# KohakuBlueleaf/UwUDiff

Measured on AMD Instinct MI355X. Metric: train images/sec (whole node), DiT-S/2 256^2 latent, higher is better.
Workload: dtype bf16; 1 GPU; DiT-S/2 (L12 D384 h6), 4x32x32 synthetic latents + pooled-text cond 1280, eps-MSE, AdamW lr1e-6 wd0.01 cosine; random-init weights; per_gpu_batch=768, global_batch=768, parallelism=dp1

## Files before the change

uwudiff_amd/csrc/attention_p256.hip:

```cpp
#include "common.h"

namespace {

constexpr int P_RING = 3;
template <int DH>
struct PGeom {
  static constexpr bool TAIL = DH > 64;
  static constexpr int SLOT = 16384 + (TAIL ? 2048 + 256 : 0);
  static constexpr int OFF_TT = 16384, OFF_TL = 16384 + 2048;
  static constexpr int OFF_DS = P_RING * SLOT;
  static constexpr int KIMG = 32768 + (TAIL ? 4096 : 0);
  static constexpr int OFF_K = OFF_DS + 32768;
  static constexpr int OFF_LSE = OFF_K + 2 * KIMG;
  static constexpr int OFF_DELTA = OFF_LSE + (TAIL ? 0 : 2 * 1024);
  static constexpr int OFF_ZERO = OFF_DELTA + 2 * 256;
  static constexpr int LDS = OFF_ZERO + (TAIL ? 16 : 0);
};
static_assert(PGeom<64>::LDS == 150016 && PGeom<72>::LDS <= 163840, "LDS budget");
constexpr int P_LDS = PGeom<64>::LDS;

struct PArgs {
  const bf16_t *q, *k, *v, *o, *dO;
  bf16_t *dq, *dk, *dv;
  const float* lse;
  int B, H, ldq, ldk, ldv, ldo, nheads;
  float scale;
};

__device__ __forceinline__ int fsw(int row) {
  return (((row >> 2) ^ (row >> 4)) & 1) | ((((row >> 3) ^ (row >> 4)) & 1) << 1) | (((row >> 1) & 1) << 2);
}
__device__ __forceinline__ int Fsw(int row) {
  return (row & 1) | (((row >> 2) & 1) << 1) | (((row >> 3) & 1) << 2) | (((row >> 1) & 1) << 3);
}

typedef short s16x4 __attribute__((ext_vector_type(4)));
typedef unsigned su32x2 __attribute__((ext_vector_type(2)));

__device__ __forceinline__ void glds16(const void* gsrc, unsigned lds_dst ) {
  unsigned keep;
  asm volatile("s_mov_b32 %0, m0\n\ts_mov_b32 m0, %2\n\ts_nop 0\n\tglobal_load_lds_dwordx4 %1, off\n\ts_mov_b32 m0, %0"
               : "=&s"(keep)
               : "v"(gsrc), "s"(lds_dst)
               : "memory");
}
__device__ __forceinline__ void glds4(const void* gsrc, unsigned lds_dst ) {
  unsigned keep;
  asm volatile("s_mov_b32 %0, m0\n\ts_mov_b32 m0, %2\n\ts_nop 0\n\tglobal_load_lds_dword %1, off\n\ts_mov_b32 m0, %0"
               : "=&s"(keep)
               : "v"(gsrc), "s"(lds_dst)
               : "memory");
}
__device__ __forceinline__ void glds16_s(const void* sbase , unsigned voff, unsigned lds_dst ) {
  unsigned keep;
  asm volatile("s_mov_b32 %0, m0\n\ts_mov_b32 m0, %3\n\ts_nop 0\n\tglobal_load_lds_dwordx4 %1, %2\n\ts_mov_b32 m0, %0"
               : "=&s"(keep)
               : "v"(voff), "s"(sbase), "s"(lds_dst)
               : "memory");
}
__device__ __forceinline__ f32x16 mfma32(const uint4& a, const uint4& b, f32x16 c) {
  return __builtin_amdgcn_mfma_f32_32x32x16_bf16(*reinterpret_cast<const bf16x8*>(&a), *reinterpret_cast<const bf16x8*>(&b), c, 0,
                                                 0, 0);
}
__device__ __forceinline__ f32x4 mfma16(const uint4& a, const uint4& b, f32x4 c) {
  return __builtin_amdgcn_mfma_f32_16x16x32_bf16(*reinterpret_cast<const bf16x8*>(&a), *reinterpret_cast<const bf16x8*>(&b), c, 0,
                                                 0, 0);
}
__device__ __forceinline__ uint4 pack8(const f32x16& x, int s) {
  bf16x8 f;
#pragma unroll
  for (int j = 0; j < 8; ++j) f[j] = (bf16_t)x[8 * s + j];
  return *reinterpret_cast<uint4*>(&f);
}

extern __shared__ __attribute__((aligned(16))) char p_smem[];

__device__ __forceinline__ void lane_halves(float x, float& lo, float& hi) {
  float a = x, b = x;
  asm volatile("v_nop\n\tv_nop\n\tv_permlane32_swap_b32 %0, %1" : "+v"(a), "+v"(b));
  lo = a;
  hi = b;
}

__device__ __forceinline__ uint4 tr_pair(unsigned a0, unsigned a1) {
  const s16x4 lo = __builtin_amdgcn_ds_read_tr16_b64_v4i16(
      (__attribute__((address_space(3))) s16x4*)((__attribute__((address_space(3))) char*)p_smem + a0));
  const s16x4 hi = __builtin_amdgcn_ds_read_tr16_b64_v4i16(
      (__attribute__((address_space(3))) s16x4*)((__attribute__((address_space(3))) char*)p_smem + a1));
  uint4 r;
  r.x = ((unsigned)(unsigned short)lo[0]) | ((unsigned)(unsigned short)lo[1] << 16);
  r.y = ((unsigned)(unsigned short)lo[2]) | ((unsigned)(unsigned short)lo[3] << 16);
  r.z = ((unsigned)(unsigned short)hi[0]) | ((unsigned)(unsigned short)hi[1] << 16);
  r.w = ((unsigned)(unsigned short)hi[2]) | ((unsigned)(unsigned short)hi[3] << 16);
  return r;
}

template <int DH>
__global__ void __launch_bounds__(512, 2) attn_bwd_p256(const PArgs a) {
  using G = PGeom<DH>;
  constexpr bool TAIL = G::TAIL;
  constexpr int T = 256, NKS = TAIL ? 5 : 4, NDT = TAIL ? 3 : 2;
  constexpr int P_SLOT = G::SLOT, P_OFF_DS = G::OFF_DS, P_OFF_K = G::OFF_K, P_OFF_LSE = G::OFF_LSE, P_OFF_DELTA = G::OFF_DELTA;
  constexpr int KIMG = G::KIMG;
  char* const smem = p_smem;
  const int tid = threadIdx.x, lane = tid & 63;
  const int wave = __builtin_amdgcn_readfirstlane(tid >> 6);
  const int r = lane & 31, h = lane >> 5;
  const int fr = lane & 15, fq = lane >> 4;
  const unsigned smem_base = (unsigned)(size_t)((const __attribute__((address_space(3))) char*)p_smem);
  const float c = a.scale * 1.4426950408889634f;
  const float ninv_scale = -1.f / a.scale;
  const int nmy = (a.nheads - (int)blockIdx.x + (int)gridDim.x - 1) / (int)gridDim.x;
  const int total = 4 * nmy;
  const int k0 = wave * 32;

  const int drow = tid >> 3;
  const int dchunk = (tid & 7) ^ fsw(drow);
  unsigned B0, A0, K0, D0, TQ0, TA0, KT0;
  auto phase1_consts = [&](int ln) {
    const int r_ = ln & 31, h_ = ln >> 5;
    B0 = (unsigned)(r_ * 128 + ((h_ ^ fsw(r_)) << 4));
    const int rowL = 4 * h_ + ((ln & 15) >> 2), chunkL = 2 * ((ln >> 4) & 1) + ((ln & 3) >> 1);
    A0 = (unsigned)(rowL * 128 + ((chunkL ^ fsw(rowL)) << 4) + 8 * (ln & 1));
    TQ0 = (unsigned)((r_ >> 3) * 256 + (r_ & 7) * 16);
    TA0 = (unsigned)(rowL * 16 + 8 * (ln & 1));
  };
  auto phase2_consts = [&](int ln) {
    const int fr_ = ln & 15, fq_ = ln >> 4;
    const int rowK = 8 * fq_ + (fr_ >> 2);
    K0 = (unsigned)(rowK * 128 + ((((fr_ & 3) >> 1) ^ fsw(rowK)) << 4) + 8 * (fr_ & 1));
    D0 = (unsigned)(rowK * 128 + (((fr_ & 3) ^ Fsw(rowK)) << 3));
    KT0 = (unsigned)(rowK * 16 + 8 * (fr_ & 1));
  };
  auto opaque_lane = [&]() {
    int ln = lane;
    asm volatile("" : "+v"(ln));
    return ln;
  };
  auto my_tid = [&]() {
    int x = tid;
    if constexpr (TAIL) asm volatile("" : "+v"(x));
    return x;
  };
  if constexpr (!TAIL) {
    phase1_consts(lane);
    phase2_consts(lane);
  }

  auto head_ptrs = [&](int j, int& b, int& hd) {
    const int bh = (int)blockIdx.x + j * (int)gridDim.x;
    b = bh / a.H;
    hd = bh - b * a.H;
  };
  uint4 oreg;
  unsigned otail = 0;
  auto issue_tile = [&](int g) {
    int b, hd;
    head_ptrs(g >> 2, b, hd);
    const int tid = my_tid(), lane = tid & 63, drow = tid >> 3, dchunk = (tid & 7) ^ fsw(drow);
    const int row = 64 * (g & 3) + drow;
    const bf16_t* qs = a.q + ((int64_t)b * T + row) * a.ldq + hd * DH + 8 * dchunk;
    const bf16_t* gs = a.dO + ((int64_t)b * T + row) * a.ldo + hd * DH + 8 * dchunk;
    const unsigned dst = smem_base + (unsigned)((g % P_RING) * P_SLOT + wave * 1024);
    glds16(qs, dst);
    glds16(gs, dst + 8192);
    oreg = *reinterpret_cast<const uint4*>(a.o + ((int64_t)b * T + row) * a.ldo + hd * DH + 8 * dchunk);
    if constexpr (TAIL) {
      const unsigned slot = smem_base + (unsigned)((g % P_RING) * P_SLOT);
      if (lane < 16) {
        const int64_t trow = (int64_t)b * T + 64 * (g & 3) + 8 * wave + (lane & 7);
        const bf16_t* src = lane < 8 ? a.q + trow * a.ldq + hd * DH + 64 : a.dO + trow * a.ldo + hd * DH + 64;
        glds16(src, slot + (unsigned)(G::OFF_TT + wave * 256));
      }
      glds4(a.lse + ((int64_t)b * a.H + hd) * T + 64 * (g & 3) + lane, slot + (unsigned)G::OFF_TL);
      otail = *reinterpret_cast<const unsigned*>(a.o + ((int64_t)b * T + row) * a.ldo + hd * DH + 64 + 2 * (tid & 3));
    }
  };
  auto issue_head = [&](int j) {
    int b, hd;
    head_ptrs(j, b, hd);
    const int tid = my_tid(), lane = tid & 63, drow = tid >> 3, dchunk = (tid & 7) ^ fsw(drow);
    const unsigned dst = smem_base + (unsigned)(P_OFF_K + (j & 1) * KIMG + wave * 1024);
#pragma unroll
    for (int p = 0; p < 4; ++p)
      glds16(a.k + ((int64_t)b * T + 64 * p + drow) * a.ldk + hd * DH + 8 * dchunk, dst + p * 8192);
    if constexpr (TAIL) {
      if (lane < 32)
        glds16(a.k + ((int64_t)b * T + 32 * wave + lane) * a.ldk + hd * DH + 64,
               smem_base + (unsigned)(P_OFF_K + (j & 1) * KIMG + 32768 + wave * 512));
    } else {
      glds4(a.lse + ((int64_t)b * a.H + hd) * T + 64 * (wave & 3) + lane,
            smem_base + (unsigned)(P_OFF_LSE + (j & 1) * 1024 + (wave & 3) * 256));
    }
  };
  uint4 kf[NKS], vf[NKS];
  auto load_kv = [&](int j) {
    int b, hd;
    head_ptrs(j, b, hd);
    const int tid = my_tid(), r = tid & 31, h = (tid >> 5) & 1;
#pragma unroll
    for (int s = 0; s < 4; ++s) {
      kf[s] = *reinterpret_cast<const uint4*>(a.k + ((int64_t)b * T + k0 + r) * a.ldk + hd * DH + 16 * s + 8 * h);
      vf[s] = *reinterpret_cast<const uint4*>(a.v + ((int64_t)b * T + k0 + r) * a.ldv + hd * DH + 16 * s + 8 * h);
    }
    if constexpr (TAIL) {
      kf[4] = *reinterpret_cast<const uint4*>(a.k + ((int64_t)b * T + k0 + r) * a.ldk + hd * DH + 64);
      vf[4] = *reinterpret_cast<const uint4*>(a.v + ((int64_t)b * T + k0 + r) * a.ldv + hd * DH + 64);
    }
  };
  auto delta_of = [&](int g) {
    const uint4 gch = *reinterpret_cast<const uint4*>(smem + (g % P_RING) * P_SLOT + 8192 + 16 * tid);
    const bf16x8 gv = *reinterpret_cast<const bf16x8*>(&gch), ov = *reinterpret_cast<const bf16x8*>(&oreg);
    float ds = 0.f;
#pragma unroll
    for (int e = 0; e < 8; ++e) ds += (float)gv[e] * (float)ov[e];
    if constexpr (TAIL) {
      const unsigned gtc = *reinterpret_cast<const unsigned*>(smem + (g % P_RING) * P_SLOT + G::OFF_TT + (drow >> 3) * 256 + 128 +
                                                              (drow & 7) * 16 + 4 * (tid & 3));
      const bf16x2 gt2 = *reinterpret_cast<const bf16x2*>(&gtc), ot2 = *reinterpret_cast<const bf16x2*>(&otail);
      const float dt2 = (float)gt2[0] * (float)ot2[0] + (float)gt2[1] * (float)ot2[1];
      ds += (tid & 4) ? 0.f : dt2;
    }
    ds += __builtin_bit_cast(float, __builtin_amdgcn_update_dpp(0, __builtin_bit_cast(int, ds), 0xB1, 0xF, 0xF, true));
    ds += __builtin_bit_cast(float, __builtin_amdgcn_update_dpp(0, __builtin_bit_cast(int, ds), 0x4E, 0xF, 0xF, true));
    ds += __builtin_bit_cast(float, __builtin_amdgcn_update_dpp(0, __builtin_bit_cast(int, ds), 0x141, 0xF, 0xF, true));
    if ((tid & 7) == 0) reinterpret_cast<float*>(smem + P_OFF_DELTA + (g & 1) * 256)[drow] = -ds;
  };

  f32x16 dkT[2], dvT[2];
  f32x4 dkt = {0.f, 0.f, 0.f, 0.f}, dvt = {0.f, 0.f, 0.f, 0.f};
#pragma unroll
  for (int dt = 0; dt < 2; ++dt) dkT[dt] = dvT[dt] = f32x16{};

  auto store_dkdv = [&](int j) {
    int b, hd;
    head_ptrs(j, b, hd);
    const int tid = my_tid(), lane = tid & 63, r = tid & 31, h = (tid >> 5) & 1;
    char* mine = smem + P_OFF_K + (j & 1) * KIMG + wave * 4096;
    char* mine_t = smem + P_OFF_K + (j & 1) * KIMG + 32768 + wave * 512;
#pragma unroll
    for (int which = 0; which < 2; ++which) {
#pragma unroll
      for (int dt = 0; dt < 2; ++dt)
#pragma unroll
        for (int g4 = 0; g4 < 4; ++g4) {
          const int d0 = 32 * dt + 8 * g4 + 4 * h;
          const f32x16& x = which ? dvT[dt] : dkT[dt];
          const float sc = which ? 1.f : a.scale;
          store4(reinterpret_cast<bf16_t*>(mine + r * 128 + (((d0 >> 3) ^ (r & 7)) << 4) + 2 * (d0 & 7)),
                 f32x4{x[4 * g4] * sc, x[4 * g4 + 1] * sc, x[4 * g4 + 2] * sc, x[4 * g4 + 3] * sc});
        }
      bf16_t* dst = (which ? a.dv : a.dk) + (int64_t)b * T * (which ? a.ldv : a.ldk) + hd * DH;
      const int ld = which ? a.ldv : a.ldk;
#pragma unroll
      for (int p = 0; p < 4; ++p) {
        const int key = 8 * p + (lane >> 3), ch = lane & 7;
        const uint4 x = *reinterpret_cast<const uint4*>(mine + key * 128 + ((ch ^ (key & 7)) << 4));
        *reinterpret_cast<uint4*>(dst + (int64_t)(k0 + key) * ld + 8 * ch) = x;
      }
      if constexpr (TAIL) {
        const f32x4 x = which ? dvt : dkt;
        const float sc = which ? 1.f : a.scale;
        store4(reinterpret_cast<bf16_t*>(mine_t + r * 16 + 8 * h), f32x4{x[0] * sc, x[1] * sc, x[2] * sc, x[3] * sc});
        const uint4 xt = *reinterpret_cast<const uint4*>(mine_t + r * 16);
        *reinterpret_cast<uint4*>(dst + (int64_t)(k0 + r) * ld + 64) = xt;
      }
    }
#pragma unroll
    for (int dt = 0; dt < 2; ++dt) dkT[dt] = dvT[dt] = f32x16{};
    dkt = dvt = f32x4{0.f, 0.f, 0.f, 0.f};
  };

  if (total == 0) return;
  if constexpr (TAIL)
    if (tid < 4) reinterpret_cast<unsigned*>(smem + G::OFF_ZERO)[tid] = 0u;
  issue_head(0);
  issue_tile(0);
  load_kv(0);
  __builtin_amdgcn_s_waitcnt(0x0070);
  asm volatile("" ::: "memory");
  __builtin_amdgcn_s_barrier();
  delta_of(0);
  if (1 < total) issue_tile(1);
  __builtin_amdgcn_s_waitcnt(0x0070);
  for (int g = 0; g < total; ++g) {
    const int j = g >> 2, t = g & 3;
    __builtin_amdgcn_s_waitcnt(TAIL ? 0x0072 : 0x0071);
    asm volatile("" ::: "memory");
    __builtin_amdgcn_s_barrier();
    if (t == 0 && j > 0) store_dkdv(j - 1);
    if (g + 1 < total) delta_of(g + 1);
    if (g + 2 < total) {
      issue_tile(g + 2);
      if (((g + 2) & 3) == 0) issue_head((g + 2) >> 2);
    }
    if constexpr (TAIL) phase1_consts(opaque_lane());
    const unsigned Qs = (unsigned)((g % P_RING) * P_SLOT), Gs = Qs + 8192;
    const float* ls = TAIL ? reinterpret_cast<const float*>(smem + (g % P_RING) * P_SLOT + G::OFF_TL)
                           : reinterpret_cast<const float*>(smem + P_OFF_LSE + (j & 1) * 1024) + 64 * t;
    const float* dl = reinterpret_cast<const float*>(smem + P_OFF_DELTA + (g & 1) * 256);
    char* const dsimg = smem + P_OFF_DS;
#pragma unroll
    for (int sub = 0; sub < 2; ++sub) {
      f32x16 S, dP;
#pragma unroll
      for (int g4 = 0; g4 < 4; ++g4) {
        const f32x4 l4 = load4(ls + 32 * sub + 8 * g4 + 4 * h);
        const f32x4 d4 = load4(dl + 32 * sub + 8 * g4 + 4 * h);
#pragma unroll
        for (int e = 0; e < 4; ++e) {
          S[4 * g4 + e] = l4[e] * ninv_scale;
          dP[4 * g4 + e] = d4[e];
        }
      }
#pragma unroll
      for (int s = 0; s < 4; ++s) {
        const unsigned off = (B0 ^ (unsigned)(s << 5)) + 4096u * sub;
        const uint4 qa = *reinterpret_cast<const uint4*>(smem + Qs + off);
        const uint4 ga = *reinterpret_cast<const uint4*>(smem + Gs + off);
        S = mfma32(qa, kf[s], S);
        dP = mfma32(ga, vf[s], dP);
      }
      if constexpr (TAIL) {
        const unsigned off = Qs + (unsigned)G::OFF_TT + TQ0 + 1024u * sub;
        const uint4 qa = *reinterpret_cast<const uint4*>(smem + (h ? (unsigned)G::OFF_ZERO : off));
        const uint4 ga = *reinterpret_cast<const uint4*>(smem + (h ? (unsigned)G::OFF_ZERO : off + 128));
        S = mfma32(qa, kf[4], S);
        dP = mfma32(ga, vf[4], dP);
      }
#pragma unroll
      for (int i = 0; i < 16; ++i) {
        const float p = __builtin_amdgcn_exp2f(S[i] * c);
        S[i] = p;
        dP[i] *= p;
      }
      bf16x2 dsp[8];
#pragma unroll
      for (int jj = 0; jj < 8; ++jj) dsp[jj] = bf16x2{(bf16_t)dP[2 * jj], (bf16_t)dP[2 * jj + 1]};
#pragma unroll
      for (int g4 = 0; g4 < 4; ++g4) {
        uint2 w;
        w.x = *reinterpret_cast<const unsigned*>(&dsp[2 * g4]);
        w.y = *reinterpret_cast<const unsigned*>(&dsp[2 * g4 + 1]);
        const int key = k0 + r;
        *reinterpret_cast<uint2*>(dsimg + key * 128 + (((8 * sub + 2 * g4 + h) ^ Fsw(key)) << 3)) = w;
      }
      f32x16 tv = {}, tk = {};
#pragma unroll
      for (int s2 = 0; s2 < 2; ++s2) {
        const uint4 pf = pack8(S, s2);
        uint4 dsf;
        dsf.x = *reinterpret_cast<const unsigned*>(&dsp[4 * s2]);
        dsf.y = *reinterpret_cast<const unsigned*>(&dsp[4 * s2 + 1]);
        dsf.z = *reinterpret_cast<const unsigned*>(&dsp[4 * s2 + 2]);
        dsf.w = *reinterpret_cast<const unsigned*>(&dsp[4 * s2 + 3]);
#pragma unroll
        for (int dt = 0; dt < 2; ++dt) {
          const unsigned x0 = (A0 ^ (unsigned)(0x30 * s2) ^ (unsigned)(0x40 * dt)) + 2048u * s2 + 4096u * sub;
          const unsigned x1 = (x0 ^ 0x20u) + 1024u;
          const uint4 gt = tr_pair(Gs + x0, Gs + x1);
          const uint4 qt = tr_pair(Qs + x0, Qs + x1);
          dvT[dt] = mfma32(gt, pf, dvT[dt]);
          dkT[dt] = mfma32(qt, dsf, dkT[dt]);
        }
        if constexpr (TAIL) {
          const unsigned x0 = Qs + (unsigned)G::OFF_TT + TA0 + 512u * s2 + 1024u * sub;
          const uint4 gt = tr_pair(x0 + 128u, x0 + 128u + 256u);
          const uint4 qt = tr_pair(x0, x0 + 256u);
          tv = mfma32(gt, pf, tv);
          tk = mfma32(qt, dsf, tk);
        }
      }
      if constexpr (TAIL) {
#pragma unroll
        for (int e = 0; e < 4; ++e) {
          dvt[e] += tv[e];
          dkt[e] += tk[e];
        }
      }
    }
    if (t == 3 && j + 1 < nmy) load_kv(j + 1);
    asm volatile("s_waitcnt lgkmcnt(0)" ::: "memory");
    __builtin_amdgcn_s_barrier();
    if constexpr (TAIL) phase2_consts(opaque_lane());
    const int qblk = wave & 3, db0 = 2 * (wave >> 2);
    const unsigned Ki = (unsigned)(P_OFF_K + (j & 1) * KIMG), Di = (unsigned)P_OFF_DS;
    const unsigned ka = K0 ^ (unsigned)(db0 << 5), kb = K0 ^ (unsigned)((db0 + 1) << 5), da = D0 ^ (unsigned)(qblk << 5);
    f32x4 acc0 = {0.f, 0.f, 0.f, 0.f}, acc1 = {0.f, 0.f, 0.f, 0.f}, acc2 = {0.f, 0.f, 0.f, 0.f};
#pragma unroll
    for (int kk = 0; kk < 8; ++kk) {
      const unsigned ko = 4096u * kk;
      const uint4 fa = tr_pair(Ki + ka + ko, Ki + (ka ^ 0x10u) + 512u + ko);
      const uint4 fb = tr_pair(Ki + kb + ko, Ki + (kb ^ 0x10u) + 512u + ko);
      const uint4 fd = tr_pair(Di + da + ko, Di + (da ^ 0x10u) + 512u + ko);
      acc0 = mfma16(fa, fd, acc0);
      acc1 = mfma16(fb, fd, acc1);
      if constexpr (TAIL) {
        const unsigned kt = Ki + 32768u + KT0 + 512u * kk;
        acc2 = mfma16(tr_pair(kt, kt + 64u), fd, acc2);
      }
    }
    int b, hd;
    head_ptrs(j, b, hd);
    const f32x4 v0 = acc0 * a.scale, v1 = acc1 * a.scale;
    const bf16x4 p0b = {(bf16_t)v0[0], (bf16_t)v0[1], (bf16_t)v0[2], (bf16_t)v0[3]};
    const bf16x4 p1b = {(bf16_t)v1[0], (bf16_t)v1[1], (bf16_t)v1[2], (bf16_t)v1[3]};
    const uint2 p0 = *reinterpret_cast<const uint2*>(&p0b), p1 = *reinterpret_cast<const uint2*>(&p1b);
    const su32x2 sx = __builtin_amdgcn_permlane16_swap(p0.x, p1.x, false, false);
    const su32x2 sy = __builtin_amdgcn_permlane16_swap(p0.y, p1.y, false, false);
    const bool odd = fq & 1;
    const int d = odd ? 16 * (db0 + 1) + 4 * (fq - 1) : 16 * db0 + 4 * fq;
    bf16_t* dst = a.dq + ((int64_t)b * T + 64 * t + 16 * qblk + fr) * a.ldq + hd * DH + d;
    *reinterpret_cast<uint4*>(dst) = uint4{sx[0], sy[0], sx[1], sy[1]};
    if constexpr (TAIL) {
      const f32x4 v2 = acc2 * a.scale;
      store4(a.dq + ((int64_t)b * T + 64 * t + 16 * qblk + fr) * a.ldq + hd * DH + 64 + 4 * (fq & 1), v2);
    }
  }
  asm volatile("s_waitcnt lgkmcnt(0)" ::: "memory");
  __builtin_amdgcn_s_barrier();
  store_dkdv(nmy - 1);
}

template <int DH>
struct FGeom {
  static constexpr bool TAIL = DH > 64;
  static constexpr int RING = TAIL ? 4 : 5;
  static constexpr int SLOT = 16384 + (TAIL ? 2048 : 0);
  static constexpr int OFF_TT = 16384;
  static constexpr int OST = 4096 + (TAIL ? 512 : 0);
  static constexpr int OFF_O = RING * SLOT;
  static constexpr int OFF_Q = OFF_O + 8 * OST;
  static constexpr int OFF_ZERO = OFF_Q + 32768 + (TAIL ? 4096 : 0);
  static constexpr int LDS = OFF_ZERO + (TAIL ? 16 : 0);
};
static_assert(FGeom<64>::LDS == 147456 && FGeom<72>::LDS <= 163840, "LDS budget");
constexpr int F_LDS = FGeom<64>::LDS;

struct FArgs {
  const bf16_t *q, *k, *v;
  bf16_t* out;
  float* lse;
  int B, H, ldq, ldk, ldv, ldo, nheads;
  float scale;
};

template <int N>
__device__ __forceinline__ void wait_vm_n() {
  asm volatile("s_waitcnt vmcnt(%0)" ::"n"(N) : "memory");
}
__device__ __forceinline__ void wait_vm(int n) {
  switch (n < 20 ? n : 20) {
    case 20: wait_vm_n<20>(); break;
    case 19: wait_vm_n<19>(); break;
    case 18: wait_vm_n<18>(); break;
    case 17: wait_vm_n<17>(); break;
    case 16: wait_vm_n<16>(); break;
    case 15: wait_vm_n<15>(); break;
    case 14: wait_vm_n<14>(); break;
    case 13: wait_vm_n<13>(); break;
    case 12: wait_vm_n<12>(); break;
    case 11: wait_vm_n<11>(); break;
    case 10: wait_vm_n<10>(); break;
    case 9: wait_vm_n<9>(); break;
    case 8: wait_vm_n<8>(); break;
    case 7: wait_vm_n<7>(); break;
    case 6: wait_vm_n<6>(); break;
    case 5: wait_vm_n<5>(); break;
    case 4: wait_vm_n<4>(); break;
    case 3: wait_vm_n<3>(); break;
    case 2: wait_vm_n<2>(); break;
    case 1: wait_vm_n<1>(); break;
    default: wait_vm_n<0>();
  }
}

template <int DH>
__global__ void __launch_bounds__(512, 2) attn_fwd_p256(const FArgs a) {
  using G = FGeom<DH>;
  constexpr bool TAIL = G::TAIL;
  constexpr int T = 256, NKS = TAIL ? 5 : 4, NDT = TAIL ? 3 : 2;
  constexpr int F_RING = G::RING, AHEAD = F_RING - 1, F_SLOT = G::SLOT, F_OFF_O = G::OFF_O, F_OFF_Q = G::OFF_Q;
  constexpr int TILE_OPS = TAIL ? 3 : 2, Q_OPS = TAIL ? 5 : 4, ST_OPS = TAIL ? 6 : 5;
  char* const smem = p_smem;
  const int tid = threadIdx.x, lane = tid & 63;
  const int wave = __builtin_amdgcn_readfirstlane(tid >> 6);
  const int r = lane & 31, h = lane >> 5;
  const unsigned smem_base = (unsigned)(size_t)((const __attribute__((address_space(3))) char*)p_smem);
  const float c = a.scale * 1.4426950408889634f;
  const int nmy = (a.nheads - (int)blockIdx.x + (int)gridDim.x - 1) / (int)gridDim.x;
  const int total = 4 * nmy;
  const int q0 = wave * 32;
  const int drow = tid >> 3;
  const int dchunk = (tid & 7) ^ fsw(drow);
  const unsigned B0 = (unsigned)(r * 128 + ((h ^ fsw(r)) << 4));
  const unsigned QR0 = (unsigned)(F_OFF_Q + (q0 + r) * 128 + ((h ^ fsw(q0 + r)) << 4));
  const int rowL = 4 * h + ((lane & 15) >> 2), chunkL = 2 * ((lane >> 4) & 1) + ((lane & 3) >> 1);
  const unsigned A0 = (unsigned)(rowL * 128 + ((chunkL ^ fsw(rowL)) << 4) + 8 * (lane & 1));
  const unsigned TQ0 = (unsigned)((r >> 3) * 256 + (r & 7) * 16);
  const unsigned TA0 = (unsigned)(rowL * 16 + 8 * (lane & 1));
  auto head_ptrs = [&](int j, int& b, int& hd) {
    const int bh = (int)blockIdx.x + j * (int)gridDim.x;
    b = bh / a.H;
    hd = bh - b * a.H;
  };
  const unsigned kvoff = (unsigned)((drow * a.ldk + 8 * dchunk) * 2), vvoff = (unsigned)((drow * a.ldv + 8 * dchunk) * 2);
  const unsigned qvoff = (unsigned)((drow * a.ldq + 8 * dchunk) * 2);
  const bf16_t *kb_n = nullptr, *vb_n = nullptr, *qb_n = nullptr;
  int b_c = 0, hd_c = 0;
  auto set_issue_head = [&](int j) {
    int b, hd;
    head_ptrs(j, b, hd);
    kb_n = a.k + (int64_t)b * T * a.ldk + hd * DH;
    vb_n = a.v + (int64_t)b * T * a.ldv + hd * DH;
    qb_n = a.q + (int64_t)b * T * a.ldq + hd * DH;
  };
  auto issue_tile = [&](int g) {
    const int t64 = 64 * (g & 3);
    const unsigned dst = smem_base + (unsigned)((g % F_RING) * F_SLOT + wave * 1024);
    glds16_s(kb_n, kvoff + (unsigned)(t64 * a.ldk * 2), dst);
    glds16_s(vb_n, vvoff + (unsigned)(t64 * a.ldv * 2), dst + 8192);
    if constexpr (TAIL) {
      if (lane < 16) {
        const int trow = t64 + 8 * wave + (lane & 7);
        const bf16_t* src = lane < 8 ? kb_n + (int64_t)trow * a.ldk + 64 : vb_n + (int64_t)trow * a.ldv + 64;
        glds16(src, smem_base + (unsigned)((g % F_RING) * F_SLOT + G::OFF_TT + wave * 256));
      }
    }
  };
  auto issue_q = [&]() {
#pragma unroll
    for (int p = 0; p < 4; ++p)
      glds16_s(qb_n, qvoff + (unsigned)(64 * p * a.ldq * 2), smem_base + (unsigned)(F_OFF_Q + p * 8192 + wave * 1024));
    if constexpr (TAIL) {
      if (lane < 32) glds16(qb_n + (int64_t)(32 * wave + lane) * a.ldq + 64, smem_base + (unsigned)(F_OFF_Q + 32768 + wave * 512));
    }
  };
  auto extras = [&](int i) { return ((i & 3) == 1 && (i >> 2) + 1 < nmy ? Q_OPS : 0) + ((i & 3) == 3 ? ST_OPS : 0); };
  auto younger = [&](int g) {
    int y = 0;
    const int gi = g - (F_RING - 1);
    if (gi < 0) {
      for (int x = g + 1; x < F_RING - 1; ++x) y += x < total ? TILE_OPS : 0;
    } else {
      y += extras(gi);
    }
    for (int i = gi < 0 ? 0 : gi + 1; i < g; ++i) y += (i + F_RING - 1 < total ? TILE_OPS : 0) + extras(i);
    return y;
  };
  if (total == 0) return;
  static_assert(AHEAD == 4 || AHEAD == 3, "the tile issued in iteration g belongs to the next head from t = 4 - AHEAD on");
  if constexpr (TAIL)
    if (tid < 4) reinterpret_cast<unsigned*>(smem + G::OFF_ZERO)[tid] = 0u;
  set_issue_head(0);
  head_ptrs(0, b_c, hd_c);
  issue_q();
#pragma unroll
  for (int g = 0; g < F_RING - 1; ++g) issue_tile(g);

  uint4 qf[NKS];
  f32x16 o[NDT];
  float m = -INFINITY, l = 0.f;
  for (int g = 0; g < total; ++g) {
    const int j = g >> 2, t = g & 3;
    int n_fly = younger(g);
    if (t == 0 && j > 0) {
      const int yq = (g - 2 + F_RING - 1 < total ? TILE_OPS : 0) + (g - 1 + F_RING - 1 < total ? TILE_OPS : 0) + ST_OPS;
      n_fly = yq < n_fly ? yq : n_fly;
    }
    wait_vm(n_fly);
    __builtin_amdgcn_s_barrier();
    if (t == 0) head_ptrs(j, b_c, hd_c);
    if (t == 4 - AHEAD && j + 1 < nmy) set_issue_head(j + 1);
    if (g + F_RING - 1 < total) issue_tile(g + F_RING - 1);
    if (t == 0) {
#pragma unroll
      for (int s = 0; s < 4; ++s) qf[s] = *reinterpret_cast<const uint4*>(smem + (QR0 ^ (unsigned)(s << 5)));
      if constexpr (TAIL)
        qf[4] = *reinterpret_cast<const uint4*>(smem + (h ? (unsigned)G::OFF_ZERO : (unsigned)(F_OFF_Q + 32768 + (q0 + r) * 16)));
#pragma unroll
      for (int dt = 0; dt < NDT; ++dt) o[dt] = f32x16{};
      m = -INFINITY;
      l = 0.f;
    }
    if (t == 1 && j + 1 < nmy) issue_q();
    const unsigned Ks = (unsigned)((g % F_RING) * F_SLOT), Vs = Ks + 8192;
    f32x16 s[2];
#pragma unroll
    for (int kt = 0; kt < 2; ++kt) {
      s[kt] = f32x16{};
#pragma unroll
      for (int ss = 0; ss < 4; ++ss) {
        const uint4 kfr = *reinterpret_cast<const uint4*>(smem + Ks + (B0 ^ (unsigned)(ss << 5)) + 4096u * kt);
        s[kt] = mfma32(kfr, qf[ss], s[kt]);
      }
      if constexpr (TAIL) {
        const uint4 kfr = *reinterpret_cast<const uint4*>(smem + Ks + (unsigned)G::OFF_TT + TQ0 + 1024u * kt);
        s[kt] = mfma32(kfr, qf[4], s[kt]);
      }
    }
    float mx = s[0][0];
#pragma unroll
    for (int kt = 0; kt < 2; ++kt)
#pragma unroll
      for (int i = 0; i < 16; ++i) mx = fmaxf(mx, s[kt][i]);
    {
      float lo, hi;
      lane_halves(mx, lo, hi);
      mx = fmaxf(lo, hi);
    }
    const float mn = fmaxf(m, mx);
    const float alpha = __builtin_amdgcn_exp2f((m - mn) * c);
    const float mc = mn * c;
    float ls = 0.f;
#pragma unroll
    for (int kt = 0; kt < 2; ++kt)
#pragma unroll
      for (int i = 0; i < 16; ++i) {
        const float p = __builtin_amdgcn_exp2f(s[kt][i] * c - mc);
        s[kt][i] = p;
        ls += p;
      }
    l = l * alpha + ls;
    m = mn;
#pragma unroll
    for (int dt = 0; dt < 2; ++dt)
#pragma unroll
      for (int i = 0; i < 16; ++i) o[dt][i] *= alpha;
    if constexpr (TAIL) {
#pragma unroll
      for (int i = 0; i < 4; ++i) o[2][i] *= alpha;
    }
#pragma unroll
    for (int kt = 0; kt < 2; ++kt)
#pragma unroll
      for (int s2 = 0; s2 < 2; ++s2) {
        const uint4 pf = pack8(s[kt], s2);
#pragma unroll
        for (int dt = 0; dt < 2; ++dt) {
          const unsigned x0 = (A0 ^ (unsigned)(0x30 * s2) ^ (unsigned)(0x40 * dt)) + 2048u * s2 + 4096u * kt;
          const uint4 vt = tr_pair(Vs + x0, Vs + (x0 ^ 0x20u) + 1024u);
          o[dt] = mfma32(vt, pf, o[dt]);
        }
        if constexpr (TAIL) {
          const unsigned x0 = Ks + (unsigned)G::OFF_TT + 128u + TA0 + 512u * s2 + 1024u * kt;
          o[2] = mfma32(tr_pair(x0, x0 + 256u), pf, o[2]);
        }
      }
    if (t == 3) {
      const int b = b_c, hd = hd_c;
      float lt;
      {
        float lo, hi;
        lane_halves(l, lo, hi);
        lt = lo + hi;
      }
      const float inv = 1.f / lt;
      char* mine = smem + F_OFF_O + wave * G::OST;
#pragma unroll
      for (int dt = 0; dt < 2; ++dt)
#pragma unroll
        for (int g4 = 0; g4 < 4; ++g4) {
          const int d0 = 32 * dt + 8 * g4 + 4 * h;
          store4(reinterpret_cast<bf16_t*>(mine + r * 128 + (((d0 >> 3) ^ (r & 7)) << 4) + 2 * (d0 & 7)),
                 f32x4{o[dt][4 * g4] * inv, o[dt][4 * g4 + 1] * inv, o[dt][4 * g4 + 2] * inv, o[dt][4 * g4 + 3] * inv});
        }
      bf16_t* ob = a.out + ((int64_t)b * T + q0) * a.ldo + hd * DH;
#pragma unroll
      for (int p = 0; p < 4; ++p) {
        const int row = 8 * p + (lane >> 3), ch = lane & 7;
        const uint4 x = *reinterpret_cast<const uint4*>(mine + row * 128 + ((ch ^ (row & 7)) << 4));
        *reinterpret_cast<uint4*>(ob + (int64_t)row * a.ldo + 8 * ch) = x;
      }
      if constexpr (TAIL) {
        store4(reinterpret_cast<bf16_t*>(mine + 4096 + r * 16 + 8 * h), f32x4{o[2][0] * inv, o[2][1] * inv, o[2][2] * inv, o[2][3] * inv});
        const uint4 xt = *reinterpret_cast<const uint4*>(mine + 4096 + r * 16);
        *reinterpret_cast<uint4*>(ob + (int64_t)r * a.ldo + 64) = xt;
      }
      a.lse[((int64_t)b * a.H + hd) * T + q0 + r] = m * a.scale + __logf(lt);
    }
  }
}

}

bool uwu_attn_p256_ok(int T, int Tk, int d, int ldq, int ldk, int ldv, int ldo) {
  static UwuEnv on("UWU_ATTN_P256");
  if (on.get().is('0') || T != 256 || Tk != 256 || ldq % 8 || ldk % 8 || ldv % 8 || ldo % 8 || uwu_dev_cus() <= 0) return false;
  if (d == 64) return uwu_dev_lds_fits(P_LDS);
  static UwuEnv on72("UWU_ATTN_P256_D72");
  return d == 72 && !on72.get().is('0') && uwu_dev_lds_fits(PGeom<72>::LDS);
}

int uwu_attn_p256_bwd(const void* q, const void* k, const void* v, const void* o, const void* dO, const float* lse, void* dq,
                      void* dk, void* dv, int B, int H, int d, int ldq, int ldk, int ldv, int ldo, float scale, hipStream_t st) {
  static unsigned char done[UWU_MAX_DEV];
  const int n_cu = uwu_dev_cus();
  if (d == 72) {
    static unsigned char done72[UWU_MAX_DEV];
    if (n_cu <= 0 || !uwu_func_lds(reinterpret_cast<const void*>(attn_bwd_p256<72>), PGeom<72>::LDS, done72)) {
      uwu_set_error("attention_bwd(p256, d = 72): the device cannot give a workgroup %d bytes of LDS", (int)PGeom<72>::LDS);
      return UWU_ELAUNCH;
    }
    PArgs a{};
    a.q = (const bf16_t*)q; a.k = (const bf16_t*)k; a.v = (const bf16_t*)v; a.o = (const bf16_t*)o; a.dO = (const bf16_t*)dO;
    a.dq = (bf16_t*)dq; a.dk = (bf16_t*)dk; a.dv = (bf16_t*)dv; a.lse = lse;
    a.B = B; a.H = H; a.ldq = ldq; a.ldk = ldk; a.ldv = ldv; a.ldo = ldo; a.nheads = B * H; a.scale = scale;
    const int grid = a.nheads < n_cu ? a.nheads : n_cu;
    hipLaunchKernelGGL(attn_bwd_p256<72>, dim3(grid), dim3(512), PGeom<72>::LDS, st, a);
    UWU_LAUNCH_CHECK("attention_bwd(p256, d = 72)");
    return UWU_OK;
  }
  if (n_cu <= 0 || !uwu_func_lds(reinterpret_cast<const void*>(attn_bwd_p256<64>), P_LDS, done)) {
    uwu_set_error("attention_bwd(p256): the device cannot give a workgroup %d bytes of LDS", (int)P_LDS);
    return UWU_ELAUNCH;
  }
  PArgs a{};
  a.q = (const bf16_t*)q; a.k = (const bf16_t*)k; a.v = (const bf16_t*)v; a.o = (const bf16_t*)o; a.dO = (const bf16_t*)dO;
  a.dq = (bf16_t*)dq; a.dk = (bf16_t*)dk; a.dv = (bf16_t*)dv; a.lse = lse;
  a.B = B; a.H = H; a.ldq = ldq; a.ldk = ldk; a.ldv = ldv; a.ldo = ldo; a.nheads = B * H; a.scale = scale;
  const int grid = a.nheads < n_cu ? a.nheads : n_cu;
  hipLaunchKernelGGL(attn_bwd_p256<64>, dim3(grid), dim3(512), P_LDS, st, a);
  UWU_LAUNCH_CHECK("attention_bwd(p256)");
  return UWU_OK;
}

bool uwu_attn_p256_fwd_ok(int nheads, int T, int Tk, int d, int ldq, int ldk, int ldv, int ldo) {
  static UwuEnv on("UWU_ATTN_P256F");
  if (on.get().is('0')) return false;
  if (!on.is('1') && nheads < 1024) return false;
  if (T != 256 || Tk != 256 || ldq % 8 || ldk % 8 || ldv % 8 || ldo % 8 || uwu_dev_cus() <= 0) return false;
  if (d == 64) return uwu_dev_lds_fits(F_LDS);
  static UwuEnv on72("UWU_ATTN_P256F_D72");
  return d == 72 && !on72.get().is('0') && uwu_dev_lds_fits(FGeom<72>::LDS);
}

int uwu_attn_p256_fwd(const void* q, const void* k, const void* v, void* o, float* lse, int B, int H, int d, int ldq, int ldk, int ldv,
                      int ldo, float scale, hipStream_t st) {
  static unsigned char done[2][UWU_MAX_DEV];
  const int n_cu = uwu_dev_cus();
  const int lds = d == 72 ? FGeom<72>::LDS : F_LDS;
  const void* fn = d == 72 ? reinterpret_cast<const void*>(attn_fwd_p256<72>) : reinterpret_cast<const void*>(attn_fwd_p256<64>);
  if (n_cu <= 0 || !uwu_func_lds(fn, lds, done[d == 72])) {
    uwu_set_error("attention_fwd(p256): the device cannot give a workgroup %d bytes of LDS", lds);
    return UWU_ELAUNCH;
  }
  FArgs a{};
  a.q = (const bf16_t*)q; a.k = (const bf16_t*)k; a.v = (const bf16_t*)v; a.out = (bf16_t*)o; a.lse = lse;
  a.B = B; a.H = H; a.ldq = ldq; a.ldk = ldk; a.ldv = ldv; a.ldo = ldo; a.nheads = B * H; a.scale = scale;
  const int grid = a.nheads < n_cu ? a.nheads : n_cu;
  if (d == 72) hipLaunchKernelGGL(attn_fwd_p256<72>, dim3(grid), dim3(512), lds, st, a);
  else hipLaunchKernelGGL(attn_fwd_p256<64>, dim3(grid), dim3(512), lds, st, a);
  UWU_LAUNCH_CHECK("attention_fwd(p256)");
  return UWU_OK;
}
```

Measured before the change: 17890 images/s.

## Replace runtime vmcnt switch with compile-time jump table and add staggered wave-group schedule

Replaces the per-iteration runtime count of in-flight loads and the 21-way switch with a constexpr table of vmcnt values indexed through an inline-asm computed jump, keyed by a 4-bit class. This removes scalar loop overhead and branches before each barrier. It also adds an optional GROUPS variant in which the two halves of the waves are offset by one barrier phase to stagger their compute, but that variant runs only when UWU_ATTN_P256F_GROUPS=1. The inline asm clobbers hard-coded SGPRs s97-s99, which is fragile.

```diff
diff --git a/uwudiff_amd/csrc/attention_p256.hip b/uwudiff_amd/csrc/attention_p256.hip
--- a/uwudiff_amd/csrc/attention_p256.hip
+++ b/uwudiff_amd/csrc/attention_p256.hip
@@ -1,3 +1,4 @@
+#include "attn_p256_waits.h"
 #include "common.h"
 
 namespace {
@@ -449,33 +450,47 @@
 __device__ __forceinline__ void wait_vm_n() {
   asm volatile("s_waitcnt vmcnt(%0)" ::"n"(N) : "memory");
 }
-__device__ __forceinline__ void wait_vm(int n) {
-  switch (n < 20 ? n : 20) {
-    case 20: wait_vm_n<20>(); break;
-    case 19: wait_vm_n<19>(); break;
-    case 18: wait_vm_n<18>(); break;
-    case 17: wait_vm_n<17>(); break;
-    case 16: wait_vm_n<16>(); break;
-    case 15: wait_vm_n<15>(); break;
-    case 14: wait_vm_n<14>(); break;
-    case 13: wait_vm_n<13>(); break;
-    case 12: wait_vm_n<12>(); break;
-    case 11: wait_vm_n<11>(); break;
-    case 10: wait_vm_n<10>(); break;
-    case 9: wait_vm_n<9>(); break;
-    case 8: wait_vm_n<8>(); break;
-    case 7: wait_vm_n<7>(); break;
-    case 6: wait_vm_n<6>(); break;
-    case 5: wait_vm_n<5>(); break;
-    case 4: wait_vm_n<4>(); break;
-    case 3: wait_vm_n<3>(); break;
-    case 2: wait_vm_n<2>(); break;
-    case 1: wait_vm_n<1>(); break;
-    default: wait_vm_n<0>();
-  }
-}
-
-template <int DH>
+template <int DH, int LAG>
+__device__ __forceinline__ void wait_tile(int g , int nmy) {
+  namespace W = attn_p256_waits;
+  constexpr W::FwdStream S = W::fwd_stream(DH);
+#define UWU_CLS_COUNT(k) "n"(W::wait_count(S, LAG, (k) & 3, ((k) & 4) != 0, ((k) & 8) != 0))
+  const int cls = __builtin_amdgcn_readfirstlane((g & 3) | (g < 4 ? 4 : 0) | ((g >> 2) + 1 < nmy ? 8 : 0));
+  asm volatile(
+      "s_getpc_b64 s[98:99]\n"
+      "3:\n\t"
+      "s_lshl_b32 s97, %0, 3\n\t"
+      "s_add_u32 s97, s97, (4f-3b)&4294967295\n\t"
+      "s_add_u32 s98, s98, s97\n\t"
+      "s_addc_u32 s99, s99, 0\n\t"
+      "s_setpc_b64 s[98:99]\n"
+      "4:\n\t"
+      "s_waitcnt vmcnt(%1)\n\ts_branch 5f\n\t"
+      "s_waitcnt vmcnt(%2)\n\ts_branch 5f\n\t"
+      "s_waitcnt vmcnt(%3)\n\ts_branch 5f\n\t"
+      "s_waitcnt vmcnt(%4)\n\ts_branch 5f\n\t"
+      "s_waitcnt vmcnt(%5)\n\ts_branch 5f\n\t"
+      "s_waitcnt vmcnt(%6)\n\ts_branch 5f\n\t"
+      "s_waitcnt vmcnt(%7)\n\ts_branch 5f\n\t"
+      "s_waitcnt vmcnt(%8)\n\ts_branch 5f\n\t"
+      "s_waitcnt vmcnt(%9)\n\ts_branch 5f\n\t"
+      "s_waitcnt vmcnt(%10)\n\ts_branch 5f\n\t"
+      "s_waitcnt vmcnt(%11)\n\ts_branch 5f\n\t"
+      "s_waitcnt vmcnt(%12)\n\ts_branch 5f\n\t"
+      "s_waitcnt vmcnt(%13)\n\ts_branch 5f\n\t"
+      "s_waitcnt vmcnt(%14)\n\ts_branch 5f\n\t"
+      "s_waitcnt vmcnt(%15)\n\ts_branch 5f\n\t"
+      "s_waitcnt vmcnt(%16)\n\ts_nop 0\n"
+      "5:"
+      :
+      : "s"(cls), UWU_CLS_COUNT(0), UWU_CLS_COUNT(1), UWU_CLS_COUNT(2), UWU_CLS_COUNT(3), UWU_CLS_COUNT(4), UWU_CLS_COUNT(5),
+        UWU_CLS_COUNT(6), UWU_CLS_COUNT(7), UWU_CLS_COUNT(8), UWU_CLS_COUNT(9), UWU_CLS_COUNT(10), UWU_CLS_COUNT(11),
+        UWU_CLS_COUNT(12), UWU_CLS_COUNT(13), UWU_CLS_COUNT(14), UWU_CLS_COUNT(15)
+      : "memory", "scc", "s97", "s98", "s99");
+#undef UWU_CLS_COUNT
+}
+
+template <int DH, bool GROUPS>
 __global__ void __launch_bounds__(512, 2) attn_fwd_p256(const FArgs a) {
   using G = FGeom<DH>;
   constexpr bool TAIL = G::TAIL;
@@ -507,7 +522,6 @@
   const unsigned kvoff = (unsigned)((drow * a.ldk + 8 * dchunk) * 2), vvoff = (unsigned)((drow * a.ldv + 8 * dchunk) * 2);
   const unsigned qvoff = (unsigned)((drow * a.ldq + 8 * dchunk) * 2);
   const bf16_t *kb_n = nullptr, *vb_n = nullptr, *qb_n = nullptr;
-  int b_c = 0, hd_c = 0;
   auto set_issue_head = [&](int j) {
     int b, hd;
     head_ptrs(j, b, hd);
@@ -536,43 +550,44 @@
       if (lane < 32) glds16(qb_n + (int64_t)(32 * wave + lane) * a.ldq + 64, smem_base + (unsigned)(F_OFF_Q + 32768 + wave * 512));
     }
   };
-  auto extras = [&](int i) { return ((i & 3) == 1 && (i >> 2) + 1 < nmy ? Q_OPS : 0) + ((i & 3) == 3 ? ST_OPS : 0); };
-  auto younger = [&](int g) {
-    int y = 0;
-    const int gi = g - (F_RING - 1);
-    if (gi < 0) {
-      for (int x = g + 1; x < F_RING - 1; ++x) y += x < total ? TILE_OPS : 0;
-    } else {
-      y += extras(gi);
-    }
-    for (int i = gi < 0 ? 0 : gi + 1; i < g; ++i) y += (i + F_RING - 1 < total ? TILE_OPS : 0) + extras(i);
-    return y;
+  auto issue_body = [&](int g) {
+    if (g + AHEAD < total) issue_tile(g + AHEAD);
+    if ((g & 3) == 1 && (g >> 2) + 1 < nmy) issue_q();
+  };
+  auto bar = [&]() __attribute__((always_inline)) {
+    __builtin_amdgcn_s_barrier();
+    __builtin_amdgcn_sched_barrier(0);
   };
   if (total == 0) return;
   static_assert(AHEAD == 4 || AHEAD == 3, "the tile issued in iteration g belongs to the next head from t = 4 - AHEAD on");
+  static_assert(AHEAD == attn_p256_waits::ahead(attn_p256_waits::fwd_stream(DH)) && TILE_OPS == attn_p256_waits::fwd_stream(DH).tile_ops &&
+                    Q_OPS == attn_p256_waits::fwd_stream(DH).q_ops && ST_OPS == attn_p256_waits::fwd_stream(DH).st_ops,
+                "attn_p256_waits.h describes this kernel's stream");
   if constexpr (TAIL)
     if (tid < 4) reinterpret_cast<unsigned*>(smem + G::OFF_ZERO)[tid] = 0u;
   set_issue_head(0);
-  head_ptrs(0, b_c, hd_c);
   issue_q();
 #pragma unroll
-  for (int g = 0; g < F_RING - 1; ++g) issue_tile(g);
-
+  for (int g = 0; g < AHEAD; ++g) issue_tile(g);
+
+  const int grp = GROUPS ? wave >> 2 : 0;
   uint4 qf[NKS];
   f32x16 o[NDT];
   float m = -INFINITY, l = 0.f;
+  if constexpr (GROUPS) {
+    asm volatile("s_waitcnt lgkmcnt(0)" ::: "memory");
+    wait_tile<DH, 0>(0, nmy);
+    bar();
+    if (grp == 1) bar();
+  }
   for (int g = 0; g < total; ++g) {
     const int j = g >> 2, t = g & 3;
-    int n_fly = younger(g);
-    if (t == 0 && j > 0) {
-      const int yq = (g - 2 + F_RING - 1 < total ? TILE_OPS : 0) + (g - 1 + F_RING - 1 < total ? TILE_OPS : 0) + ST_OPS;
-      n_fly = yq < n_fly ? yq : n_fly;
-    }
-    wait_vm(n_fly);
-    __builtin_amdgcn_s_barrier();
-    if (t == 0) head_ptrs(j, b_c, hd_c);
-    if (t == 4 - AHEAD && j + 1 < nmy) set_issue_head(j + 1);
-    if (g + F_RING - 1 < total) issue_tile(g + F_RING - 1);
+    if constexpr (!GROUPS) {
+      wait_tile<DH, 0>(g, nmy);
+      __builtin_amdgcn_s_barrier();
+      if (t == 4 - AHEAD && j + 1 < nmy) set_issue_head(j + 1);
+      issue_body(g);
+    }
     if (t == 0) {
 #pragma unroll
       for (int s = 0; s < 4; ++s) qf[s] = *reinterpret_cast<const uint4*>(smem + (QR0 ^ (unsigned)(s << 5)));
@@ -583,7 +598,6 @@
       m = -INFINITY;
       l = 0.f;
     }
-    if (t == 1 && j + 1 < nmy) issue_q();
     const unsigned Ks = (unsigned)((g % F_RING) * F_SLOT), Vs = Ks + 8192;
     f32x16 s[2];
 #pragma unroll
@@ -598,6 +612,12 @@
         const uint4 kfr = *reinterpret_cast<const uint4*>(smem + Ks + (unsigned)G::OFF_TT + TQ0 + 1024u * kt);
         s[kt] = mfma32(kfr, qf[4], s[kt]);
       }
+    }
+    if constexpr (GROUPS) {
+      if (t == 4 - AHEAD && j + 1 < nmy) set_issue_head(j + 1);
+      if (grp == 1 && g + 1 < total) wait_tile<DH, 1>(g + 1, nmy);
+      bar();
+      issue_body(g);
     }
     float mx = s[0][0];
 #pragma unroll
@@ -648,7 +668,8 @@
         }
       }
     if (t == 3) {
-      const int b = b_c, hd = hd_c;
+      int b, hd;
+      head_ptrs(j, b, hd);
       float lt;
       {
         float lo, hi;
@@ -679,6 +700,14 @@
       }
       a.lse[((int64_t)b * a.H + hd) * T + q0 + r] = m * a.scale + __logf(lt);
     }
+    if constexpr (GROUPS) {
+      asm volatile("s_waitcnt lgkmcnt(0)" ::: "memory");
+      if (grp == 0 && g + 1 < total) wait_tile<DH, 0>(g + 1, nmy);
+      bar();
+    }
+  }
+  if constexpr (GROUPS) {
+    if (grp == 0) bar();
   }
 }
 
@@ -737,11 +766,15 @@
 
 int uwu_attn_p256_fwd(const void* q, const void* k, const void* v, void* o, float* lse, int B, int H, int d, int ldq, int ldk, int ldv,
                       int ldo, float scale, hipStream_t st) {
-  static unsigned char done[2][UWU_MAX_DEV];
+  static UwuEnv groups("UWU_ATTN_P256F_GROUPS");
+  static unsigned char done[4][UWU_MAX_DEV];
   const int n_cu = uwu_dev_cus();
   const int lds = d == 72 ? FGeom<72>::LDS : F_LDS;
-  const void* fn = d == 72 ? reinterpret_cast<const void*>(attn_fwd_p256<72>) : reinterpret_cast<const void*>(attn_fwd_p256<64>);
-  if (n_cu <= 0 || !uwu_func_lds(fn, lds, done[d == 72])) {
+  const int sch = groups.get().is('1') ? 1 : 0;
+  using Kern = void (*)(const FArgs);
+  static const Kern kern[2][2] = {{attn_fwd_p256<64, false>, attn_fwd_p256<64, true>}, {attn_fwd_p256<72, false>, attn_fwd_p256<72, true>}};
+  const Kern fn = kern[d == 72][sch];
+  if (n_cu <= 0 || !uwu_func_lds(reinterpret_cast<const void*>(fn), lds, done[2 * (d == 72) + sch])) {
     uwu_set_error("attention_fwd(p256): the device cannot give a workgroup %d bytes of LDS", lds);
     return UWU_ELAUNCH;
   }
@@ -749,8 +782,7 @@
   a.q = (const bf16_t*)q; a.k = (const bf16_t*)k; a.v = (const bf16_t*)v; a.out = (bf16_t*)o; a.lse = lse;
   a.B = B; a.H = H; a.ldq = ldq; a.ldk = ldk; a.ldv = ldv; a.ldo = ldo; a.nheads = B * H; a.scale = scale;
   const int grid = a.nheads < n_cu ? a.nheads : n_cu;
-  if (d == 72) hipLaunchKernelGGL(attn_fwd_p256<72>, dim3(grid), dim3(512), lds, st, a);
-  else hipLaunchKernelGGL(attn_fwd_p256<64>, dim3(grid), dim3(512), lds, st, a);
+  hipLaunchKernelGGL(fn, dim3(grid), dim3(512), lds, st, a);
   UWU_LAUNCH_CHECK("attention_fwd(p256)");
   return UWU_OK;
 }
diff --git a/uwudiff_amd/csrc/attn_p256_waits.h b/uwudiff_amd/csrc/attn_p256_waits.h
--- /dev/null
+++ b/uwudiff_amd/csrc/attn_p256_waits.h
@@ -0,0 +1,72 @@
+#pragma once
+
+namespace attn_p256_waits {
+
+struct FwdStream {
+  int ring;
+  int tile_ops;
+  int q_ops;
+  int st_ops;
+};
+constexpr FwdStream fwd_stream(int head_dim) { return head_dim > 64 ? FwdStream{4, 3, 5, 6} : FwdStream{5, 2, 4, 5}; }
+constexpr int ahead(const FwdStream& s) { return s.ring - 1; }
+
+constexpr int body_tile(const FwdStream& s, int i, int nmy) { return i + ahead(s) < 4 * nmy ? s.tile_ops : 0; }
+constexpr int body_q(const FwdStream& s, int i, int nmy) { return (i & 3) == 1 && (i >> 2) + 1 < nmy ? s.q_ops : 0; }
+constexpr int body_st(const FwdStream& s, int i) { return (i & 3) == 3 ? s.st_ops : 0; }
+
+constexpr int wait_lag(bool groups, int group) { return groups && group == 1 ? 1 : 0; }
+
+constexpr int wait_count_walk(const FwdStream& s, int lag, int g, int nmy) {
+  int seq = s.q_ops, last_awaited = (g == 0 ? seq : 0) - 1;
+  for (int x = 0; x < ahead(s); ++x) {
+    seq += s.tile_ops;
+    if (x == g) last_awaited = seq - 1;
+  }
+  for (int i = 0; i < g - lag; ++i) {
+    if (body_tile(s, i, nmy)) {
+      seq += s.tile_ops;
+      if (i + ahead(s) == g) last_awaited = seq - 1;
+    }
+    if (body_q(s, i, nmy)) {
+      seq += s.q_ops;
+      if ((g & 3) == 0 && (i >> 2) + 1 == g >> 2 && seq - 1 > last_awaited) last_awaited = seq - 1;
+    }
+    seq += body_st(s, i);
+  }
+  return seq - 1 - last_awaited;
+}
+
+constexpr int wait_count(const FwdStream& s, int lag, int t, bool first, bool not_last) {
+  const int j = first ? 0 : 1;
+  return wait_count_walk(s, lag, 4 * j + t, j + (not_last ? 2 : 1));
+}
+constexpr int wait_count_max(const FwdStream& s, int lag) {
+  int m = 0;
+  for (int c = 0; c < 16; ++c) {
+    const int v = wait_count(s, lag, c & 3, (c >> 2) & 1, (c >> 3) & 1);
+    m = v > m ? v : m;
+  }
+  return m;
+}
+
+static_assert(wait_count(fwd_stream(64), 0, 0, true, true) == 6 && wait_count(fwd_stream(64), 1, 0, true, false) == 6, "");
+static_assert(wait_count(fwd_stream(64), 0, 1, true, true) == 6 && wait_count(fwd_stream(64), 1, 1, true, true) == 4, "");
+static_assert(wait_count(fwd_stream(64), 0, 2, true, false) == 2 && wait_count(fwd_stream(64), 1, 2, true, true) == 4, "");
+static_assert(wait_count(fwd_stream(64), 0, 3, true, true) == 10 && wait_count(fwd_stream(64), 1, 3, true, false) == 0, "");
+static_assert(wait_count(fwd_stream(64), 0, 0, false, true) == 9 && wait_count(fwd_stream(64), 1, 0, false, false) == 2, "");
+static_assert(wait_count(fwd_stream(64), 0, 1, false, true) == 15 && wait_count(fwd_stream(64), 1, 1, false, true) == 13, "");
+static_assert(wait_count(fwd_stream(64), 0, 2, false, false) == 7 && wait_count(fwd_stream(64), 1, 2, false, true) == 9, "");
+static_assert(wait_count(fwd_stream(64), 0, 3, false, true) == 15 && wait_count(fwd_stream(64), 1, 3, false, false) == 5, "");
+static_assert(wait_count(fwd_stream(72), 0, 0, true, true) == 6 && wait_count(fwd_stream(72), 1, 1, true, true) == 3, "");
+static_assert(wait_count(fwd_stream(72), 0, 1, true, false) == 6 && wait_count(fwd_stream(72), 0, 2, true, true) == 11, "");
+static_assert(wait_count(fwd_stream(72), 1, 2, true, true) == 3 && wait_count(fwd_stream(72), 0, 3, true, true) == 11, "");
+static_assert(wait_count(fwd_stream(72), 0, 0, false, false) == 12 && wait_count(fwd_stream(72), 1, 0, false, true) == 3, "");
+static_assert(wait_count(fwd_stream(72), 0, 1, false, true) == 12 && wait_count(fwd_stream(72), 1, 1, false, false) == 9, "");
+static_assert(wait_count(fwd_stream(72), 0, 2, false, true) == 17 && wait_count(fwd_stream(72), 1, 2, false, true) == 9, "");
+static_assert(wait_count(fwd_stream(72), 0, 3, false, false) == 0 && wait_count(fwd_stream(72), 1, 3, false, true) == 8, "");
+static_assert(wait_count_max(fwd_stream(64), 0) == 15 && wait_count_max(fwd_stream(72), 0) == 17, "vmcnt holds 63");
+
+constexpr int barriers(bool groups, int nmy) { return groups ? 8 * nmy + 2 : 4 * nmy; }
+
+}
```

After: 17890 images/s. About the same (-0.0%).
